# nurturenature/jepsen-tigerbeetle

Measured on AMD Instinct MI355X. Metric: histories/sec, 10k-op/64-proc cas-register histories (time-to-verdict ms in extra), higher is better.
Workload: dtype u64

## Files before the change

### jepsen-tigerbeetle_amd/csrc/batch_create.hip

```cpp
#include "tbc_batch.h"
#include "reach_table.h"

using namespace tbc;

namespace tbc {

uint64_t open_list_entries(const tbc_ops& c, uint64_t op_off, uint64_t n, uint32_t n_events, uint32_t n_slots,
                                  std::vector<uint32_t>& pre, bool branch_lists) {
  const uint64_t worst = std::max<uint64_t>(n, 1) * std::max(1u, n_slots);
  if (n == 0) return 1;
  if ((uint64_t)n_events > 64 * n + 1024) return worst;
  const uint32_t* inv = c.inv_pos + op_off;
  const uint32_t* ret = c.ret_pos + op_off;
  pre.assign((size_t)n_events + 1, 0u);
  for (uint64_t i = 0; i < n; i++) {
    if (ret[i] == TBC_POS_CRASHED) continue;
    if (ret[i] >= n_events || inv[i] > ret[i]) return worst;
    pre[ret[i] + 1] = 1;
  }
  for (uint32_t x = 1; x <= n_events; x++) pre[x] += pre[x - 1];
  uint64_t total = 0;
  const uint8_t* f = c.f + op_off;
  for (uint64_t i = 0; i < n; i++)
    if (ret[i] != TBC_POS_CRASHED && !(branch_lists && f[i] == TBC_F_READ)) total += pre[ret[i]] - pre[inv[i]] + 1;
// ... 354 lines not shown
    }
  }
  if (B->sweep) { tot.bstack_n = 0; tot.btab_n = 0; }
  return TBC_OK;
}

}

void tbc_batch::count_device_bytes() {
  tbc_batch* const B = this;
  const bool beam = B->width > 1;
  B->device_bytes = B->d_f.bytes() + B->d_a.bytes() + B->d_b.bytes() + B->d_proc.bytes() + B->d_inv.bytes() +
                    B->d_ret.bytes() + B->d_hist.bytes() + B->d_rec.bytes() + B->d_seg.bytes() + B->d_ret_slot.bytes() +
                    B->d_ret_op.bytes() + B->d_bitmap.bytes() + B->d_wpre.bytes() + B->d_frames.bytes() +
                    B->d_tab.bytes() + B->d_results.bytes() + B->d_work.bytes() + B->d_witness.bytes();
  if (beam) B->device_bytes += B->d_bh.bytes() + B->d_off.bytes() + B->d_ncr.bytes() + B->d_lst.bytes() +
                               B->d_crashed.bytes() + B->d_slot8.bytes() + B->d_rk8.bytes() + B->d_twn.bytes() + B->d_rdm.bytes() + B->d_look.bytes() + B->d_looktmp.bytes() + B->d_dstack.bytes() + B->d_stack.bytes() + B->d_btab.bytes() + B->d_pool.bytes() + B->d_cmem.bytes();
  if (B->d_stage[0].p) B->device_bytes += B->d_stage[0].bytes();
  if (B->d_stage[1].p) B->device_bytes += B->d_stage[1].bytes();
}

tbc_batch::~tbc_batch() {
  tbc::stream_release(this);
  d_f.release(); d_a.release(); d_b.release(); d_proc.release(); d_inv.release(); d_ret.release();
  d_hist.release(); d_rec.release(); d_seg.release(); d_ret_slot.release(); d_ret_op.release();
  d_bitmap.release(); d_wpre.release(); d_frames.release(); d_witness.release(); d_work.release();
  d_queue.release(); d_tab.release(); d_results.release(); d_table.release(); d_pool_vals.release(); d_cfg.release();
  d_bh.release(); d_off.release(); d_ncr.release(); d_lst.release(); d_crashed.release(); d_stack.release();
  d_zncr.release(); d_reach.release(); d_reach_hdr.release(); d_abort.release(); d_order.release(); d_park.release();
  if (abort_one) (void)hipHostFree(abort_one);
  if (progress) (void)hipHostFree(progress);
  d_progress.release();
  if (!borrowed) { for (auto& e : ev2) if (e) (void)hipEventDestroy(e); if (stream2) (void)hipStreamDestroy(stream2); }
  d_cmem.release(); d_occ.release(); d_btab.release(); d_slot8.release(); d_rk8.release(); d_look.release(); d_looktmp.release(); d_twn.release(); d_rdm.release(); d_cuts.release(); d_seglist.release(); d_sres.release(); d_dstack.release(); d_pool.release(); d_pool_cursor.release();
  if (ev_turn) (void)hipEventDestroy(ev_turn);
  if (!borrowed) {
    for (auto& e : ev) if (e) (void)hipEventDestroy(e);
    if (stream) (void)hipStreamDestroy(stream);
  }
}

namespace tbc {
namespace {

tbc_status alloc_arenas(CreatePlan& P) {
  tbc_batch* B = P.B; const tbc_opts* opts = P.opts; const tbc_model* model = P.model;
  const uint32_t nh = P.nh;
  const bool beam = P.beam, device_sizing = P.device_sizing;
  const LayoutTotals& t = P.tot;
  const uint32_t EW = B->entry_words();
  tbc_status s;
  const uint64_t T = B->total_ops;
  if (!t_ctx) {
    HIP_TRY(hipHostMalloc((void**)&B->progress, 16 * sizeof(uint32_t), hipHostMallocMapped | hipHostMallocCoherent));
    std::memset(B->progress, 0, 16 * sizeof(uint32_t));
    if ((s = B->d_progress.alloc(1))) return s;
  }
  if ((s = B->d_f.alloc(T)) || (s = B->d_a.alloc(T)) || (s = B->d_b.alloc(T)) || (s = B->d_proc.alloc(T)) ||
      (s = B->d_inv.alloc(T)) || (s = B->d_ret.alloc(T)) || (s = B->d_hist.alloc(nh)) || (s = B->d_bh.alloc(beam ? nh : 0)) || (s = B->d_work.alloc(nh)) ||
      (s = B->d_bitmap.alloc(t.bm_n)) || (s = B->d_off.alloc(beam ? t.boff_n : 0)) || (s = B->d_ncr.alloc(beam ? t.boff_n : 0)) || (s = B->d_pool_cursor.alloc(1)) ||
      (s = B->d_rec.alloc(t.rec_n)) ||
      (s = B->d_seg.alloc(t.seg_n)) || (s = B->d_ret_slot.alloc(T)) || (s = B->d_ret_op.alloc(T)) ||
      (s = B->d_wpre.alloc(t.bm_n)) || (s = B->d_frames.alloc(t.frame_n)) ||
      (s = B->d_tab.alloc(t.tab_n)) || (s = B->d_results.alloc(nh)) ||
      (s = B->d_queue.alloc(4)) || (s = B->d_witness.alloc(opts->want_witness ? T : 0)))
    return s;
  if (beam) {
    if ((!device_sizing && (s = B->d_lst.alloc(t.blst_n))) || (s = B->d_crashed.alloc((B->count_form || !B->any_crashed) ? 0 : T)) || (s = B->d_cmem.alloc(B->count_form ? t.bocc_n : 0)) ||
        (s = B->d_slot8.alloc(slot8_bytes(T, nh))) || (s = B->d_stack.alloc(t.bstack_n)) || (s = B->d_btab.alloc(t.btab_n * B->tab_stride())))
      return s;
    if ((B->sweep || B->rsweep) && ((s = B->d_cuts.alloc((uint64_t)nh * B->max_segs)) || (s = B->d_sres.alloc((uint64_t)nh * B->max_segs * kSweepSlices)) || (s = B->d_seglist.alloc((uint64_t)nh * B->max_segs * kSweepSlices * 3)))) return s;
    if (B->sweep || B->rsweep) B->seg_host.resize((size_t)nh * B->max_segs * kSweepSlices);
    if (B->rsweep) {
      std::vector<uint32_t> reach, hdr;
      for (uint32_t h = 0; h < nh; h++) {
        const CountHist& ch = B->count_hist[h];
        hdr.push_back((uint32_t)reach.size());
        hdr.push_back(build_reach_table(ch.words.data(), ch.n_classes, reach));
      }
      if ((s = B->d_zncr.alloc(t.boff_n)) || (s = B->d_reach.alloc(reach.size())) || (s = B->d_reach_hdr.alloc(hdr.size())) || (s = B->d_abort.alloc(nh))) return s;
      HIP_TRY(hipMemset(B->d_zncr.p, 0, B->d_zncr.bytes()));
      HIP_TRY(hipMemcpy(B->d_reach.p, reach.data(), reach.size() * 4, hipMemcpyHostToDevice));
      HIP_TRY(hipMemcpy(B->d_reach_hdr.p, hdr.data(), hdr.size() * 4, hipMemcpyHostToDevice));
      HIP_TRY(hipHostMalloc((void**)&B->abort_one, sizeof(uint32_t), hipHostMallocDefault));
      *B->abort_one = 1u;
    }
    if (B->lanes && (s = B->d_rk8.alloc(slot8_bytes(T, nh)))) return s;
    if (B->reg_rules() && ((!device_sizing && (s = B->d_twn.alloc(t.blst_n * B->mask_words))) || (s = B->d_rdm.alloc(B->lanes ? 1 : T * B->vpad * B->mask_words)))) return s;
    if (B->lanes) { B->d_rdm.release(); if ((s = B->d_rdm.alloc(T * B->front_words()))) return s; }
    const bool by_front = B->mask_words == 1 && B->vpad <= 32;
    if (B->lookahead && ((s = B->d_look.alloc(look_words(T, nh, B->mask_words))) || (s = B->d_looktmp.alloc(by_front ? 0 : T)) ||
                         (s = B->d_dstack.alloc(t.bstack_n)))) return s;
    {
      uint64_t biggest = 0;
      for (uint32_t h = 0; h < nh; h++) biggest = std::max<uint64_t>(biggest, 1ull << B->bh[h].tab_log2);
      uint64_t words = std::max<uint64_t>(t.btab_n * B->tab_stride() * (B->lanes ? 1u : 3u) / 10, biggest * (4 + 16 + 4) * (EW + 1));
      words = std::min<uint64_t>(words, (32ull << 30) / 8);
      if (B->sweep) words = 1;
      if ((s = B->d_pool.alloc(words))) return s;
    }
  }
  if ((s = B->d_cfg.alloc((uint64_t)nh * kCfgCap * (2 + B->mask_words)))) return s;
  if (beam && (s = B->d_park.alloc((uint64_t)nh * kParkWords))) return s;
  B->pool_len = P.desc->cols.pool ? P.desc->cols.pool_len : 0;
  if ((s = B->d_pool_vals.alloc(B->pool_len))) return s;
  if (B->pool_len) HIP_TRY(hipMemcpy(B->d_pool_vals.p, P.desc->cols.pool, (size_t)B->pool_len * 4, hipMemcpyHostToDevice));
  if (model->kind == TBC_MODEL_TABLE) {
    const size_t tn = (size_t)model->n_states * model->n_classes;
    B->table_host.assign(model->table, model->table + tn);
    if ((s = B->d_table.alloc(tn))) return s;
    HIP_TRY(hipMemcpy(B->d_table.p, B->table_host.data(), tn * 2, hipMemcpyHostToDevice));
    B->model.table = nullptr;
  }
  B->count_device_bytes();
  return TBC_OK;
}

tbc_status take_streams(tbc_batch* B) {
  if (t_ctx) {
// ... 236 lines not shown
```

### jepsen-tigerbeetle_amd/csrc/batch_run.hip

```cpp
#include "tbc_batch.h"
#include "witness_expand.h"

using namespace tbc;

namespace tbc {

static SearchArgs make_search_args(tbc_batch* B, uint64_t* tab, uint32_t n_work) {
  SearchArgs a{};
  a.hist = B->d_hist.p; a.rec = B->d_rec.p; a.seg = B->d_seg.p; a.ret_slot = B->d_ret_slot.p;
  a.ret_op = B->d_ret_op.p;
  a.frames = B->d_frames.p; a.tab = tab; a.results = B->d_results.p;
  a.witness = B->opts.want_witness ? B->d_witness.p : nullptr;
  a.work = B->d_work.p; a.queue = B->d_queue.p;
  a.table = B->d_table.p; a.n_work = n_work; a.model_kind = B->model.kind;
  a.init_state = B->model.init;
  a.n_classes = B->model.n_classes; a.n_states = B->model.n_states;
  a.max_steps = B->opts.max_steps;
  a.time_limit_ticks = B->opts.time_limit_ms * 100000ull;
  a.dbg = debug_words();
  a.pool_vals = B->d_pool_vals.p;
  a.cfg = B->d_cfg.p;
  a.progress = B->progress; a.progress_dev = B->d_progress.p;
  return a;
}
// ... 293 lines not shown
    o.algorithm = TBC_ALG_COMPETITION; o.want_witness = 0; o.search_width = 0; o.lanes_per_history = 0; o.round_budget = 0; o.max_steps = 0;
    o.visited_per_op = 0; o.list_order = TBC_ORDER_DEFAULT;
    if (chunk == 1) {
      tbc_ops one = d.cols;
      one.n = (uint32_t)T; one.n_events = nev[0]; one.n_process = npr[0];
      tbc_model m1 = B->model;
      m1.init = aux[0];
      tbc_result r1;
      st = tbc_check(&one, &m1, &o, &r1);
      if (st == TBC_OK) { out[list[lo]] = r1; out[list[lo]].witness = nullptr; tbc_result_free(&r1); }
      continue;
    }
    tbc_batch* I = nullptr;
    st = tbc_batch_create(&d, &B->model, &o, &I);
    if (st == TBC_OK) {
      std::vector<tbc_result> res(k);
      st = tbc_batch_run(I, res.data());
      for (uint32_t i = 0; i < k && st == TBC_OK; i++) { out[list[lo + i]] = res[i]; out[list[lo + i]].witness = nullptr; }
      tbc_batch_destroy(I);
    }
  }
  return st;
}

namespace {

struct RunState {
  tbc_batch* const B;
  tbc_result* const results;
  const int phase;
  const uint64_t t_start;
  const uint32_t nh;
  hipStream_t const s;
  const bool beam;
  const uint32_t KW, EW;
  HostBuf<Hist>& hist_back;
  HostBuf<BeamHist>& bh_back;
  const uint64_t count_budget;
  const uint64_t restart_budget;
  uint64_t first_budget() const { return count_budget ? count_budget : restart_budget; }
  SweepArgs swa{};
  const bool stall_on;
  std::vector<tbc_result> handed;
  std::vector<uint8_t> was_handed;
  std::vector<uint32_t> rs_level;
  std::vector<uint8_t> rs_valid;
  const uint64_t max_bytes;
  std::vector<uint32_t> final_log2;
  std::vector<uint8_t> is_seq;
  std::vector<uint8_t> by_sweep;
  std::vector<uint32_t> width_of;
  std::vector<uint8_t> scratched;
  bool touched_work = false;
  static constexpr uint64_t arena_budget = 32ull << 30;

  RunState(tbc_batch* b, tbc_result* res, int ph)
      : B(b), results(res), phase(ph), t_start(now_ns()), nh(b->n_hist), s(b->stream), beam(b->width > 1), KW(1 + b->mask_words), EW(b->entry_words()),
        hist_back(b->hist_back_m), bh_back(b->bh_back_m),
        count_budget((b->count_form && b->opts.max_steps == 0) ? 32ull * b->max_ops : 0ull),
        restart_budget((ph == 0 && !b->sweep && b->order_restarts_apply()) ? 32ull * b->max_ops : 0ull),
        stall_on(b->lanes != 0 && (b->opts.dominance & TBC_DOM_STALL_HANDOVER) != 0 && !b->count_form && b->mask_words == 1 && !b->opts.want_witness && b->opts.max_steps == 0 && ph == 0 &&
                 (b->model.kind == TBC_MODEL_REGISTER || b->model.kind == TBC_MODEL_CAS_REGISTER) && b->vpad != 0),
        was_handed(b->n_hist, 0), rs_level(b->n_hist, kInf), rs_valid(b->n_hist, 0),
        max_bytes(b->opts.max_visited_bytes ? b->opts.max_visited_bytes : (1ull << 30)) {
    if (B->sweep || B->rsweep) {
      swa.hist = B->d_hist.p; swa.bh = B->d_bh.p; swa.off = B->d_off.p; swa.ncr = B->d_ncr.p; swa.lst = B->d_lst.p;
      swa.crashed = B->d_crashed.p; swa.twn = B->reg_rules() ? B->d_twn.p : nullptr; swa.rdm = B->reg_rules() ? B->d_rdm.p : nullptr;
      swa.slot8 = B->d_slot8.p; swa.cuts = B->d_cuts.p; swa.seg = B->d_sres.p; swa.table = B->d_table.p;
      swa.pool_vals = B->d_pool_vals.p; swa.n_hist = nh; swa.max_segs = B->max_segs; swa.seg_target = B->seg_target;
      swa.cut_open = B->cut_open; swa.n_dom = B->n_dom; swa.vpad = B->vpad ? B->vpad : 1; swa.rules = B->rules;
      swa.model_kind = B->model.kind; swa.init_state = B->model.init;
      swa.n_classes = B->model.n_classes; swa.n_keys = B->model.n_keys;
      swa.shard_rank = 0; swa.shard_world = 1;
    }
  }
};

tbc_status queue_pack(RunState& R) {
  tbc_batch* B = R.B; hipStream_t s = R.s; const uint32_t nh = R.nh; const bool beam = R.beam;
  bool packed = false, counted = false;
  if (nh <= 8) {
    bool fits = true, fits2 = beam;
    for (uint32_t h = 0; h < nh; h++) {
      fits = fits && pack_one_fits(B->model.kind, B->hist[h].n_ops, B->hist[h].n_events, B->hist[h].n_slots);
      fits2 = fits2 && pack_one_counts_fits(B->model.kind, B->hist[h].n_ops, B->hist[h].n_events, B->hist[h].n_slots);
    }
    if (fits2) packed = counted = launch_pack_one_counts(make_pack_args(B), make_pack_open_args(B), s);
    if (!packed && fits) packed = launch_pack_one(make_pack_args(B), s);
  }
  if (!packed && beam) {
    bool fits = true, slots64 = true;
    for (uint32_t h = 0; h < nh && fits; h++) {
      fits = pack_wg_fits(B->model.kind, B->hist[h].n_ops, B->hist[h].n_events, B->hist[h].n_slots);
      slots64 = slots64 && pack_wg64_fits(B->model.kind, B->hist[h].n_ops, B->hist[h].n_events, B->hist[h].n_slots);
    }
    if (fits) packed = counted = launch_pack_wg(make_pack_args(B), make_pack_open_args(B), s, slots64);
  }
  if (!packed) launch_pack(make_pack_args(B), s);
  HIP_TRY(hipGetLastError());
  if (beam) {
    PackOpenArgs po = make_pack_open_args(B);
    if (B->assign_lists) {
      if (!counted) { launch_open_counts(po, s); HIP_TRY(hipGetLastError()); counted = true; }
      tbc_status as = stream_assign_lists(B);
      if (as != TBC_OK) return as;
    }
    launch_pack_open(po, s, counted);
    HIP_TRY(hipGetLastError());
  }
  return TBC_OK;
}

tbc_status first_pass(RunState& R) {
  tbc_batch* B = R.B; hipStream_t s = R.s; const uint32_t nh = R.nh; const bool beam = R.beam; const int phase = R.phase;
  HostBuf<Hist>& hist_back = R.hist_back; HostBuf<BeamHist>& bh_back = R.bh_back;
  TRACE("run: begin");
  HIP_TRY(hipEventRecord(B->ev[0], s));
  if (B->d_progress.p) HIP_TRY(hipMemsetAsync(B->d_progress.p, 0, sizeof(uint32_t), s));
  const bool zero_block = B->borrowed && !guard_on() && !B->d_bitmap.owned && !B->d_off.owned && !B->d_ncr.owned && !B->d_pool_cursor.owned &&
                          (char*)B->d_bitmap.p < (char*)B->d_pool_cursor.p && (size_t)((char*)B->d_pool_cursor.p - (char*)B->d_bitmap.p) < (64u << 20) &&
                          (char*)B->d_off.p > (char*)B->d_bitmap.p && (char*)B->d_off.p < (char*)B->d_pool_cursor.p &&
                          (char*)B->d_ncr.p > (char*)B->d_bitmap.p && (char*)B->d_ncr.p < (char*)B->d_pool_cursor.p;
  const bool fresh = B->inputs_fresh;
  B->inputs_fresh = false;
  if (zero_block) HIP_TRY(hipMemsetAsync(B->d_bitmap.p, 0, (size_t)((char*)B->d_pool_cursor.p - (char*)B->d_bitmap.p) + sizeof(unsigned long long), s));
  else HIP_TRY(hipMemsetAsync(B->d_bitmap.p, 0, B->d_bitmap.bytes(), s));
  const bool use_epoch = beam && B->lanes != 0;
  if (beam) {
    if (use_epoch) B->epoch = B->epoch % 255u + 1u;
    if (!B->sweep && (!use_epoch || B->epoch == 1u)) HIP_TRY(hipMemsetAsync(B->d_btab.p, 0, B->d_btab.bytes(), s));
    if (!B->sweep) HIP_TRY(hipMemsetAsync(B->d_pool.p, 0, B->d_pool.bytes(), s));
    if (!zero_block) {
      HIP_TRY(hipMemsetAsync(B->d_pool_cursor.p, 0, sizeof(unsigned long long), s));
      HIP_TRY(hipMemsetAsync(B->d_off.p, 0, B->d_off.bytes(), s));
      HIP_TRY(hipMemsetAsync(B->d_ncr.p, 0, B->d_ncr.bytes(), s));
    }
    if (!fresh) HIP_TRY(hipMemcpyAsync(B->d_bh.p, B->bh.data(), nh * sizeof(BeamHist), hipMemcpyHostToDevice, s));
  } else {
    HIP_TRY(hipMemsetAsync(B->d_tab.p, 0, B->d_tab.bytes(), s));
  }
  if (!fresh) HIP_TRY(hipMemcpyAsync(B->d_hist.p, B->hist.data(), nh * sizeof(Hist), hipMemcpyHostToDevice, s));
  HIP_TRY(hipEventRecord(B->ev[1], s));
  TRACE("run: memsets queued");
  SYNC_TRACE("memsets");

  if (!B->hist_order.empty()) {
    if (B->d_order.n < nh) { B->d_order.release(); const tbc_status os = B->d_order.alloc(nh); if (os != TBC_OK) return os; }
    HIP_TRY(hipMemcpyAsync(B->d_order.p, B->hist_order.data(), (size_t)nh * 4, hipMemcpyHostToDevice, s));
  }
  tbc_status ps = queue_pack(R);
  if (ps != TBC_OK) return ps;
  TRACE("run: pack launched");
  SYNC_TRACE("pack");
  HIP_TRY(hipEventRecord(B->ev[2], s));

  bool rs_on = B->rsweep && phase == 0 && beam && !B->lanes;
  SweepArgs ra = R.swa;
  if (rs_on) {
    ra.ncr = B->d_zncr.p; ra.crashed = nullptr; ra.reach = B->d_reach.p; ra.reach_hdr = B->d_reach_hdr.p;
    ra.rules = B->rules & (kRuleEager | kRuleTwin);
    HIP_TRY(hipMemsetAsync(B->d_abort.p, 0, B->d_abort.bytes(), s));
    HIP_TRY(hipEventRecord(B->ev2[0], s));
    HIP_TRY(hipStreamWaitEvent(B->stream2, B->ev2[0], 0));
    hist_back.resize(nh);
    if (launch_sweep(ra, B->stream2)) {
      HIP_TRY(hipGetLastError());
      HIP_TRY(hipMemcpyAsync(B->seg_host.data(), B->d_sres.p, B->seg_host.size() * sizeof(SegResult), hipMemcpyDeviceToHost, B->stream2));
      HIP_TRY(hipMemcpyAsync(hist_back.data(), B->d_hist.p, nh * sizeof(Hist), hipMemcpyDeviceToHost, B->stream2));
    } else rs_on = false;
  }

  if (B->sweep) {
    SweepArgs mine = R.swa;
    if (phase == 1 && B->shard_world > 1) {
      mine.shard_rank = B->shard_rank; mine.shard_world = B->shard_world;
      HIP_TRY(hipMemsetAsync(B->d_sres.p, 0, B->d_sres.bytes(), s));
    }
    if (!launch_sweep(mine, s)) { set_error("level sweep launch failed"); return TBC_ERR_HIP; }
  } else if (beam) {
    BeamArgs ba = make_beam_args(B, B->d_btab.p, B->d_stack.p, B->d_dstack.p, nh);
    if (R.first_budget()) ba.max_steps = R.first_budget();
    if (rs_on) ba.abort = B->d_abort.p;
    if (B->lanes) { ba.tab_stride = B->tab_stride(); ba.epoch = use_epoch ? B->epoch : 0u; }
    if (R.stall_on) ba.stall_checks = kStallChecks;
    if (B->lanes) {
      SearchTurn turn(B->device, s);
      if (!B->ev_turn) HIP_TRY(hipEventCreate(&B->ev_turn));
      HIP_TRY(hipEventRecord(B->ev_turn, s));
      if (!launch_narrow(ba, B->mask_words, B->lanes, s, narrow_waves_per_simd())) { set_error("unsupported mask width"); return TBC_ERR_UNSUPPORTED; }
    } else if (!launch_beam(ba, B->mask_words, search_blocks(nh), s)) { set_error("unsupported mask width"); return TBC_ERR_UNSUPPORTED; }
  } else {
    SearchArgs sa = make_search_args(B, B->d_tab.p, nh);
    if (!launch_search(sa, B->mask_words, search_blocks(nh), s)) { set_error("unsupported mask width"); return TBC_ERR_UNSUPPORTED; }
  }
  HIP_TRY(hipGetLastError());
  TRACE("run: search launched");
  SYNC_TRACE("search");
  if (rs_on) {
    HIP_TRY(hipStreamSynchronize(B->stream2));
    const uint32_t SL = kSweepSlices;
    std::vector<uint32_t> again;
    for (uint32_t h = 0; h < nh; h++) if (hist_back[h].status == 0)
      for (uint32_t k = 0; k < B->max_segs; k++) for (uint32_t j = 0; j < SL; j++)
        if (B->seg_host[((size_t)h * B->max_segs + k) * SL + j].status == kSegOverflow) { again.push_back(h); again.push_back(k); again.push_back(j); }
    if (!again.empty()) {
      HIP_TRY(hipMemcpyAsync(B->d_seglist.p, again.data(), again.size() * 4, hipMemcpyHostToDevice, B->stream2));
      SweepArgs r2 = ra;
      r2.seg_list = B->d_seglist.p; r2.n_list = (uint32_t)(again.size() / 3);
      if (launch_sweep(r2, B->stream2)) {
        HIP_TRY(hipGetLastError());
        HIP_TRY(hipMemcpyAsync(B->seg_host.data(), B->d_sres.p, B->seg_host.size() * sizeof(SegResult), hipMemcpyDeviceToHost, B->stream2));
      }
      HIP_TRY(hipStreamSynchronize(B->stream2));
    }
    for (uint32_t h = 0; h < nh; h++) {
      if (hist_back[h].status != 0 || hist_back[h].n_ret == 0) continue;
      tbc_sweep_verdict v{};
      (void)tbc_sweep_compose(&B->seg_host[(size_t)h * B->max_segs * SL], B->max_segs, hist_back[h].n_ret, &v);
      if (v.valid == TBC_INVALID) {
        R.rs_level[h] = v.fail_level;
        HIP_TRY(hipMemcpyAsync(B->d_abort.p + h, B->abort_one, 4, hipMemcpyHostToDevice, B->stream2));
      }
      R.rs_valid[h] = v.valid == TBC_VALID;
    }
    TRACE("run: relaxed sweep composed");
  }
  HIP_TRY(hipEventRecord(B->ev[3], s));
  if (!B->sweep) HIP_TRY(hipMemcpyAsync(B->res_host.data(), B->d_results.p, nh * sizeof(DevResult), hipMemcpyDeviceToHost, s));
  else HIP_TRY(hipMemcpyAsync(B->seg_host.data(), B->d_sres.p, B->seg_host.size() * sizeof(SegResult), hipMemcpyDeviceToHost, s));
  hist_back.resize(nh);
  bh_back.resize(beam ? nh : 0);
  HIP_TRY(hipMemcpyAsync(hist_back.data(), B->d_hist.p, nh * sizeof(Hist), hipMemcpyDeviceToHost, s));
  if (beam) HIP_TRY(hipMemcpyAsync(bh_back.data(), B->d_bh.p, nh * sizeof(BeamHist), hipMemcpyDeviceToHost, s));
  if (B->borrowed && B->sweep) {
    const uint64_t t_spin = now_ns();
    hipError_t q;
    while ((q = hipStreamQuery(s)) == hipErrorNotReady && now_ns() - t_spin < 3000000ull) {}
    if (q != hipSuccess && q != hipErrorNotReady) HIP_TRY(q);
  }
  HIP_TRY(hipStreamSynchronize(s));
  if (rs_on) HIP_TRY(hipStreamSynchronize(B->stream2));
  TRACE("run: first pass synced");
  for (uint32_t h = 0; h < nh; h++) if (R.rs_level[h] != kInf) {
    DevResult& d = B->res_host[h];
    std::memset(&d, 0, sizeof d);
    d.valid = TBC_UNKNOWN; d.cause = TBC_CAUSE_STEP_LIMIT; d.fail_op = TBC_NO_OP; d.prev_ok_op = TBC_NO_OP; d.final_state = B->model.init;
    d.tab_log2 = B->bh[h].tab_log2;
  }
  return TBC_OK;
}

tbc_status sweep_verdicts(RunState& R) {
  tbc_batch* B = R.B; hipStream_t s = R.s; const uint32_t nh = R.nh;
  HostBuf<Hist>& hist_back = R.hist_back; HostBuf<BeamHist>& bh_back = R.bh_back;
  const SweepArgs& swa = R.swa;
  const uint32_t SL = kSweepSlices;
  {
    std::vector<uint32_t> again;
    for (uint32_t h = 0; h < nh; h++) if (hist_back[h].status == 0 && bh_back[h].status == 0)
      for (uint32_t k = 0; k < B->max_segs; k++) for (uint32_t j = 0; j < SL; j++)
        if (B->seg_host[((size_t)h * B->max_segs + k) * SL + j].status == kSegOverflow) { again.push_back(h); again.push_back(k); again.push_back(j); }
    if (!again.empty()) {
      HIP_TRY(hipMemcpyAsync(B->d_seglist.p, again.data(), again.size() * 4, hipMemcpyHostToDevice, s));
      SweepArgs sa2 = swa;
      sa2.seg_list = B->d_seglist.p; sa2.n_list = (uint32_t)(again.size() / 3);
      if (launch_sweep(sa2, s)) {
        HIP_TRY(hipGetLastError());
        HIP_TRY(hipMemcpyAsync(B->seg_host.data(), B->d_sres.p, B->seg_host.size() * sizeof(SegResult), hipMemcpyDeviceToHost, s));
      }
      HIP_TRY(hipStreamSynchronize(s));
    }
  }
  std::vector<uint32_t> fb, lg;
  for (uint32_t h = 0; h < nh; h++) {
    DevResult& d = B->res_host[h];
    std::memset(&d, 0, sizeof d);
    d.fail_op = TBC_NO_OP; d.prev_ok_op = TBC_NO_OP; d.final_state = B->model.init;
    if (hist_back[h].status != 0) { d.valid = TBC_UNKNOWN; continue; }
    if (hist_back[h].n_ret == 0) { d.valid = TBC_VALID; R.by_sweep[h] = 1; continue; }
    const SegResult* sg = &B->seg_host[(size_t)h * B->max_segs * SL];
    tbc_sweep_verdict v{};
    (void)tbc_sweep_compose(sg, B->max_segs, hist_back[h].n_ret, &v);
    const bool give_up = bh_back[h].status != 0 || v.valid == TBC_UNKNOWN;
    const uint32_t fail_seg = v.valid == TBC_INVALID ? v.fail_seg : kInf, fail_level = v.fail_level;
    const bool ended = v.valid == TBC_VALID;
    const uint32_t* live_in = v.live_in;
    d.steps = v.probes; d.probes = v.probes; d.visited = v.configs_total; d.backtracks = v.subrounds; d.max_depth = v.max_level;
    if (std::getenv("TBC_DEBUG")) {
      uint32_t longest = 0; uint64_t maxp = 0;
      for (uint32_t q = 0; q < B->max_segs * SL; q++) if (sg[q].status == kSegOk) { longest = std::max(longest, sg[q].F1 - sg[q].F0); maxp = std::max<uint64_t>(maxp, sg[q].probes); }
      std::fprintf(stderr, "[tbc sweep] history %u: %u wavefronts, longest segment %u levels, most probes in one %llu, largest level %llu, verdict %d\n",
                   h, v.n_wavefronts, longest, (unsigned long long)maxp, (unsigned long long)v.max_level, v.valid);
    }
    if (give_up || (fail_seg == kInf && !ended)) { fb.push_back(h); lg.push_back(B->bh[h].tab_log2); continue; }
    R.by_sweep[h] = 1;
// ... 146 lines not shown
  }
  return TBC_OK;
}

static const uint32_t kRestartOrders[] = {16u + 48u, 2u, 1u, 16u + 8u, 0u};

static const uint32_t kRaceOrders[] = {16u + 48u, 2u, 1u, 16u + 8u, 0u};
tbc_status race_orders(RunState& R, const std::vector<uint32_t>& pend_all) {
  tbc_batch* B = R.B; const uint32_t nh = R.nh; hipStream_t s = R.s;
  constexpr uint32_t K = sizeof(kRaceOrders) / sizeof(kRaceOrders[0]);
  const uint32_t default_order = B->list_order();
  R.handed.resize(nh);
  B->last_raced = (uint32_t)pend_all.size();
  CtxSuspend own_arenas;
  size_t mem_free = 0, mem_total = 0;
  if (hipMemGetInfo(&mem_free, &mem_total) != hipSuccess) mem_free = 32ull << 30;
  const uint64_t mem_cap = std::max<uint64_t>(8ull << 30, (uint64_t)mem_free / 4 * 3);
  std::vector<DevResult> outer_res(nh);
  size_t lo = 0;
  while (lo < pend_all.size()) {
    uint64_t ops = 0;
    size_t hi = lo;
    while (hi < pend_all.size() && (hi == lo || (ops + B->hist[pend_all[hi]].n_ops) * 4000ull * (K + 1) <= mem_cap)) { ops += B->hist[pend_all[hi]].n_ops; hi++; }
    const uint32_t k = (uint32_t)(hi - lo);
    std::vector<uint32_t> res_list, outer_map(nh, 0u);
    for (uint32_t i = 0; i < k; i++) {
      const uint32_t h = pend_all[lo + i];
      outer_map[h] = i;
      if (!R.scratched[h] && B->d_park.p) res_list.push_back(h);
    }
    DevBuf<uint32_t> decided, d_outer_map, d_inner_map;
    tbc_status st;
    if ((st = decided.alloc(k)) || (st = d_outer_map.alloc(nh))) return st;
    HIP_TRY(hipMemsetAsync(decided.p, 0, (size_t)k * 4, s));
    HIP_TRY(hipMemcpyAsync(d_outer_map.p, outer_map.data(), (size_t)nh * 4, hipMemcpyHostToDevice, s));
    std::vector<uint32_t> rep_hist, rep_order;
    for (uint32_t i = 0; i < k; i++) {
      for (uint32_t o : kRaceOrders) if (o != default_order) { rep_hist.push_back(i); rep_order.push_back(o); }
      if (R.scratched[pend_all[lo + i]] || !B->d_park.p) { rep_hist.push_back(i); rep_order.push_back(default_order); }
    }
    const uint32_t nr = (uint32_t)rep_hist.size();
    FetchedColumns fc;
    if ((st = fetch_columns(B, pend_all.data() + lo, k, fc)) != TBC_OK) return st;
    const std::vector<uint64_t>& goff = fc.off;
    const uint8_t* const gf = fc.f; const int32_t* const ga = fc.a; const int32_t* const gb = fc.b; const int32_t* const gp = fc.proc;
    const uint32_t* const gi = fc.inv; const uint32_t* const gr = fc.ret;
    const uint32_t n_res = (uint32_t)res_list.size();
    if (n_res) {
      HIP_TRY(hipMemcpyAsync(B->d_work.p, res_list.data(), (size_t)n_res * 4, hipMemcpyHostToDevice, s));
      BeamArgs ba = make_beam_args(B, B->d_btab.p, B->d_stack.p, B->d_dstack.p, n_res);
      ba.resume = 1; ba.max_steps = 0; ba.abort = decided.p; ba.abort_set = decided.p; ba.abort_map = d_outer_map.p;
      if (!launch_beam(ba, B->mask_words, search_blocks(n_res), s)) { set_error("unsupported mask width"); return TBC_ERR_UNSUPPORTED; }
      HIP_TRY(hipGetLastError());
      R.touched_work = true;
    }
    std::vector<uint64_t> off(nr + 1, 0);
    std::vector<uint32_t> nev(nr), npr(nr), imap(nr);
    for (uint32_t r = 0; r < nr; r++) {
      const Hist& H = B->hist[pend_all[lo + rep_hist[r]]];
      off[r + 1] = off[r] + H.n_ops; nev[r] = H.n_events; npr[r] = H.n_slots; imap[r] = rep_hist[r];
    }
    const uint64_t T = off[nr];
    if (T > 0xFFFFFFFFull) { set_error("the race's replicas exceed 2^32 ops"); return TBC_ERR_OOM; }
    std::vector<uint8_t> f(T + 1);
    std::vector<int32_t> a(T + 1), b(T + 1), pr(T + 1);
    std::vector<uint32_t> inv(T + 1), ret(T + 1);
    for (uint32_t r = 0; r < nr; r++) {
      const uint64_t n = off[r + 1] - off[r], o = off[r], g0 = goff[rep_hist[r]];
      std::memcpy(f.data() + o, gf + g0, n);
      std::memcpy(a.data() + o, ga + g0, n * 4); std::memcpy(b.data() + o, gb + g0, n * 4); std::memcpy(pr.data() + o, gp + g0, n * 4);
      std::memcpy(inv.data() + o, gi + g0, n * 4); std::memcpy(ret.data() + o, gr + g0, n * 4);
    }
    tbc_batch_desc d{};
    d.n_hist = nr; d.op_off = off.data(); d.n_events = nev.data(); d.n_process = npr.data();
    d.cols.n = (uint32_t)T; d.cols.f = f.data(); d.cols.a = a.data(); d.cols.b = b.data(); d.cols.process = pr.data();
    d.cols.inv_pos = inv.data(); d.cols.ret_pos = ret.data();
    tbc_opts o = B->opts;
    o.algorithm = TBC_ALG_COMPETITION; o.want_witness = 0; o.search_width = B->width; o.lanes_per_history = 64; o.round_budget = 0; o.max_steps = 0;
    o.visited_per_op = 64; o.list_order = TBC_ORDER_SLOT; o.dominance = (B->opts.dominance | TBC_DOM_NO_ORDER_RESTARTS) & ~TBC_DOM_STALL_HANDOVER;
    std::vector<tbc_result> res(nr);
    tbc_batch* inner = nullptr;
    TRACE("race: the replicas' batch is being made");
    st = nr ? tbc_batch_create(&d, &B->model, &o, &inner) : TBC_OK;
    if (st == TBC_OK && nr) {
      st = d_inner_map.alloc(nr);
      if (st == TBC_OK && hipMemcpy(d_inner_map.p, imap.data(), (size_t)nr * 4, hipMemcpyHostToDevice) != hipSuccess) st = TBC_ERR_HIP;
      if (st == TBC_OK) {
        inner->ext_abort = decided.p; inner->ext_abort_set = decided.p; inner->ext_abort_map = d_inner_map.p;
        inner->hist_order = rep_order;
        TRACE("race: the replicas run");
        st = tbc_batch_run(inner, res.data());
        TRACE("race: the replicas are done");
      }
    }
    if (inner) tbc_batch_destroy(inner);
    HIP_TRY(hipSetDevice(B->device));
    const bool inner_ok = nr != 0 && (st == TBC_OK || st == TBC_ERR_BAD_HISTORY || st == TBC_ERR_MODEL);
    if (!inner_ok && n_res == 0) { decided.release(); d_outer_map.release(); d_inner_map.release(); return st == TBC_OK ? TBC_ERR_HIP : st; }
    if (n_res) HIP_TRY(hipMemcpyAsync(outer_res.data(), B->d_results.p, (size_t)nh * sizeof(DevResult), hipMemcpyDeviceToHost, s));
    HIP_TRY(hipStreamSynchronize(s));
    TRACE("race: the resumed default order is done");
    decided.release(); d_outer_map.release(); d_inner_map.release();
    std::vector<uint32_t> first_rep(k, 0xFFFFFFFFu);
    for (uint32_t r = nr; r-- > 0;) first_rep[rep_hist[r]] = r;
    for (uint32_t i = 0; i < k; i++) {
      const uint32_t h = pend_all[lo + i];
// ... 325 lines not shown
```

### jepsen-tigerbeetle_amd/csrc/tbc_batch.h

```cpp
#pragma once
#include <hip/hip_runtime.h>
#include <algorithm>
#include <atomic>
#include <chrono>
#include <cstdio>
#include <cstdlib>
#include <cstring>
#include <deque>
#include <mutex>
#include <new>
#include <thread>
#include <vector>
#include "tbc_internal.h"

namespace tbc {

#define HIP_TRY(expr)                                                             \
  do {                                                                            \
    hipError_t e_ = (expr);                                                       \
    if (e_ != hipSuccess) {                                                       \
      ::tbc::set_error("%s failed: %s (%s:%d)", #expr, hipGetErrorString(e_), __FILE__, __LINE__); \
      return e_ == hipErrorOutOfMemory ? TBC_ERR_OOM : TBC_ERR_HIP;               \
    }                                                                             \
  } while (0)

inline uint32_t ceil_log2(uint64_t x) {
  uint32_t l = 0;
  while ((1ull << l) < x) l++;
  return l;
}

uint64_t now_ns();
bool device_is_gfx950(int dev);
uint32_t* debug_words();
#define SYNC_TRACE(msg) do { if (std::getenv("TBC_SYNC_EACH")) { hipError_t e__ = hipStreamSynchronize(s); std::fprintf(stderr, "[tbc sync] %s -> %s\n", msg, hipGetErrorString(e__)); std::fflush(stderr); } } while (0)
#define TRACE(msg) do { if (std::getenv("TBC_DEBUG")) { std::fprintf(stderr, "[tbc %9.3f ms] %s\n", (double)(::tbc::now_ns() % 100000000000ull) / 1e6, msg); std::fflush(stderr); } } while (0)

struct Ctx {
  int device = 0;
  char* slab = nullptr;
  size_t cap = 0, used = 0, wanted = 0;
  char* pin = nullptr;
  size_t pin_cap = 0, pin_used = 0, pin_wanted = 0;
  hipStream_t stream = nullptr;
  hipEvent_t ev[6] = {};
  hipStream_t stream2 = nullptr;
  hipEvent_t ev2[2] = {};
};
extern thread_local Ctx* t_ctx;
Ctx* ctx_acquire(int device);
void ctx_release(Ctx* c);
struct CtxSuspend {
  Ctx* const saved;
  CtxSuspend() : saved(t_ctx) { t_ctx = nullptr; }
  ~CtxSuspend() { t_ctx = saved; }
};

bool guard_on();
constexpr size_t kGuardBytes = 256;
extern thread_local const void* t_guard_owner;
extern thread_local size_t t_guard_nth;
void guard_add(const void* arena_end);
void guard_remove(const void* arena_end);
size_t guard_check(const char* when, const void* owner);

template <typename T>
// ... 130 lines not shown
  std::vector<uint32_t> hist_order;
  tbc::DevBuf<uint32_t> d_order;
  tbc::DevBuf<uint32_t> d_park;
  uint32_t last_raced = 0;
  uint32_t* progress = nullptr;
  tbc::DevBuf<uint32_t> d_progress;
  mutable std::atomic<uint32_t> progress_seen{0};
  std::atomic<uint64_t> run_t0{0};
  std::atomic<uint32_t> running{0};
  bool order_restarts_apply() const {
    return width > 1 && !lanes && !count_form && list_order_applies() && opts.list_order == TBC_ORDER_DEFAULT && opts.max_steps == 0 &&
           !(opts.dominance & TBC_DOM_NO_ORDER_RESTARTS);
  }
  std::vector<tbc::BeamHist> bh;
  tbc::DevBuf<tbc::BeamHist> d_bh;
  tbc::DevBuf<uint32_t> d_off, d_ncr, d_stack;
  tbc::DevBuf<tbc::OpRec> d_lst, d_crashed;
  tbc::DevBuf<uint8_t> d_slot8;
  tbc::DevBuf<uint8_t> d_rk8;
  bool lookahead = false;
  tbc::DevBuf<uint64_t> d_look;
  tbc::DevBuf<uint32_t> d_dstack;
  tbc::DevBuf<uint32_t> d_looktmp;
  bool sweep = false;
  uint32_t max_segs = 1, seg_target = 0, cut_open = 0, n_dom = 1;
  tbc::DevBuf<uint32_t> d_cuts, d_seglist;
  tbc::DevBuf<tbc::SegResult> d_sres;
  tbc::HostBuf<tbc::SegResult> seg_host;
  bool rsweep = false;
  tbc::DevBuf<uint32_t> d_zncr, d_reach, d_reach_hdr, d_abort;
  hipStream_t stream2 = nullptr;
  hipEvent_t ev2[2] = {};
  uint32_t* abort_one = nullptr;
  uint32_t last_segments = 0, last_fallback = 0;
  uint32_t shard_rank = 0, shard_world = 1;
  bool partial_done = false;
  tbc::HostBuf<tbc::Hist> hist_back_m;
  tbc::HostBuf<tbc::BeamHist> bh_back_m;
  tbc::HostBuf<char> upload_stage;
  bool inputs_fresh = false;
  uint32_t rules = 0;
  uint32_t vpad = 0;
  tbc::DevBuf<uint64_t> d_twn, d_rdm;
  tbc::DevBuf<uint64_t> d_occ, d_btab, d_pool;
  bool count_form = false;
  tbc::DevBuf<uint64_t> d_cmem;
  std::vector<tbc::CountHist> count_hist;
  uint32_t reg_rules() const { return rules & (tbc::kRuleEager | tbc::kRuleTwin); }
  uint32_t epoch = 0;
  bool any_crashed = true;
  uint32_t tab_stride() const { return entry_words() - ((lanes && !opts.want_witness) ? 1u : 0u); }
  uint32_t entry_words() const { return mask_words + 2u + (count_form ? tbc::kCountWords : 0u); }
  tbc::DevBuf<unsigned long long> d_pool_cursor;
  std::vector<tbc::DevResult> res_host;
  std::vector<uint32_t> witness_host;
  uint64_t timing_ns[4] = {0, 0, 0, 0};
  hipEvent_t ev_turn = nullptr;
  uint64_t turn_wait_ns = 0;
  tbc_counters sum{};
  uint64_t device_bytes = 0;
  void count_device_bytes();

  struct InputSlot { char* mem = nullptr; size_t bytes = 0; hipEvent_t copied = nullptr; bool busy = false; uint32_t* planned = nullptr; };
  std::vector<InputSlot> in_slots;
  uint32_t in_hist_cap = 0;
  uint64_t in_ops_cap = 0;
  tbc::DevBuf<uint32_t> d_stage[2];
  hipStream_t stream_copy = nullptr;
  hipEvent_t ev_stage[2] = {};
  hipEvent_t ev_unpacked[2] = {};
  bool stage_used[2] = {false, false};
  uint64_t in_seq = 0;
  std::deque<tbc_pending_input> pending;
  tbc::DevBuf<uint32_t> d_in_flags;
  uint32_t* in_flags_host = nullptr;
  bool assign_lists = false;
  tbc::DevBuf<uint32_t> d_list_over;
  uint64_t in_bytes_copied = 0, in_copy_ns = 0;
  hipEvent_t ev_copy[2][2] = {};
  tbc::LayoutTotals cap;
  bool lists_headroom = false;
  bool inputs_stale = false;
  uint64_t inputs_consumed = 0;
  uint32_t lists_regrown = 0, reload_slot = 0;

  bool borrowed = false;
  ~tbc_batch();
};

namespace tbc {

struct ColumnScan { bool nonneg = true, any_crashed = false, any_crashed_effect = false; int32_t vmax = -1; };
ColumnScan scan_columns(const tbc_ops& c, uint64_t T);
tbc_status layout_histories(tbc_batch* B, uint32_t nh, const uint64_t* op_off, const uint32_t* n_events, const uint32_t* n_slots, const int32_t* aux,
                            const uint32_t* list_caps, bool lists_on_device, std::vector<Hist>& hist, std::vector<BeamHist>& bh, LayoutTotals& tot,
                            const std::vector<CountHist>* count_hist = nullptr);
bool build_count_form(const tbc_ops& c, uint64_t o0, uint64_t n, uint32_t n_process, bool cas_model, int32_t* slot_col, CountHist& out,
                      std::vector<uint32_t>& rets, std::vector<int32_t>& slot_of, std::vector<uint8_t>& used);
uint64_t open_list_entries(const tbc_ops& c, uint64_t op_off, uint64_t n, uint32_t n_events, uint32_t n_slots, std::vector<uint32_t>& pre, bool branch_lists);
tbc_status batch_create_impl(const tbc_batch_desc* desc, const tbc_model* model, const tbc_opts* opts, tbc_batch* B);

PackArgs make_pack_args(tbc_batch* B);
PackOpenArgs make_pack_open_args(tbc_batch* B);
tbc_status batch_run_impl(tbc_batch* B, tbc_result* results, int phase = 0);

tbc_status stream_consume(tbc_batch* B, bool* consumed);
// ... 6 lines not shown
```

Baseline: 380,400.

## Trim per-pass device memsets using memoized pool usage and dirty tracking

Replaces the unconditional per-run memsets of the bitmap, offsets, ncr and visited pool with a planner. The bitmap and offsets are cleared only when the pack kernel does not already overwrite them. ncr is cleared only when the previous pass may have dirtied it. The pool is cleared only up to the cursor value read back from the previous pass. The progress word now lives next to the pool cursor, so a single memset resets both. This cuts redundant device fill bandwidth and launch count, at the cost of extra host-side state that must be kept correct across timeouts, races and arena changes.

```diff
diff --git a/jepsen-tigerbeetle_amd/csrc/batch_create.hip b/jepsen-tigerbeetle_amd/csrc/batch_create.hip
--- a/jepsen-tigerbeetle_amd/csrc/batch_create.hip
+++ b/jepsen-tigerbeetle_amd/csrc/batch_create.hip
@@ -430,19 +430,20 @@
   tbc_status s;
   const uint64_t T = B->total_ops;
   if (!t_ctx) {
-    HIP_TRY(hipHostMalloc((void**)&B->progress, 16 * sizeof(uint32_t), hipHostMallocMapped | hipHostMallocCoherent));
-    std::memset(B->progress, 0, 16 * sizeof(uint32_t));
-    if ((s = B->d_progress.alloc(1))) return s;
+    HIP_TRY(hipHostMalloc((void**)&B->progress, 18 * sizeof(uint32_t), hipHostMallocMapped | hipHostMallocCoherent));
+    std::memset(B->progress, 0, 18 * sizeof(uint32_t));
+    B->pool_used_host = reinterpret_cast<unsigned long long*>(B->progress + 16);
   }
   if ((s = B->d_f.alloc(T)) || (s = B->d_a.alloc(T)) || (s = B->d_b.alloc(T)) || (s = B->d_proc.alloc(T)) ||
       (s = B->d_inv.alloc(T)) || (s = B->d_ret.alloc(T)) || (s = B->d_hist.alloc(nh)) || (s = B->d_bh.alloc(beam ? nh : 0)) || (s = B->d_work.alloc(nh)) ||
-      (s = B->d_bitmap.alloc(t.bm_n)) || (s = B->d_off.alloc(beam ? t.boff_n : 0)) || (s = B->d_ncr.alloc(beam ? t.boff_n : 0)) || (s = B->d_pool_cursor.alloc(1)) ||
+      (s = B->d_bitmap.alloc(t.bm_n)) || (s = B->d_off.alloc(beam ? t.boff_n : 0)) || (s = B->d_ncr.alloc(beam ? t.boff_n : 0)) || (s = B->d_pool_cursor.alloc(t_ctx ? 1 : 2)) ||
       (s = B->d_rec.alloc(t.rec_n)) ||
       (s = B->d_seg.alloc(t.seg_n)) || (s = B->d_ret_slot.alloc(T)) || (s = B->d_ret_op.alloc(T)) ||
       (s = B->d_wpre.alloc(t.bm_n)) || (s = B->d_frames.alloc(t.frame_n)) ||
       (s = B->d_tab.alloc(t.tab_n)) || (s = B->d_results.alloc(nh)) ||
       (s = B->d_queue.alloc(4)) || (s = B->d_witness.alloc(opts->want_witness ? T : 0)))
     return s;
+  if (!t_ctx) { B->d_progress.p = reinterpret_cast<uint32_t*>(B->d_pool_cursor.p + 1); B->d_progress.n = 1; B->d_progress.owned = false; B->d_progress.guarded = false; }
   if (beam) {
     if ((!device_sizing && (s = B->d_lst.alloc(t.blst_n))) || (s = B->d_crashed.alloc((B->count_form || !B->any_crashed) ? 0 : T)) || (s = B->d_cmem.alloc(B->count_form ? t.bocc_n : 0)) ||
         (s = B->d_slot8.alloc(slot8_bytes(T, nh))) || (s = B->d_stack.alloc(t.bstack_n)) || (s = B->d_btab.alloc(t.btab_n * B->tab_stride())))
diff --git a/jepsen-tigerbeetle_amd/csrc/batch_run.hip b/jepsen-tigerbeetle_amd/csrc/batch_run.hip
--- a/jepsen-tigerbeetle_amd/csrc/batch_run.hip
+++ b/jepsen-tigerbeetle_amd/csrc/batch_run.hip
@@ -369,6 +369,7 @@
   std::vector<uint32_t> width_of;
   std::vector<uint8_t> scratched;
   bool touched_work = false;
+  bool block_zeroed = false;
   static constexpr uint64_t arena_budget = 32ull << 30;
 
   RunState(tbc_batch* b, tbc_result* res, int ph)
@@ -413,8 +414,11 @@
     }
     if (fits) packed = counted = launch_pack_wg(make_pack_args(B), make_pack_open_args(B), s, slots64);
   }
+  const PackFills pf = plan_pack_fills(R.block_zeroed, beam, packed, counted);
+  if (pf.bitmap) HIP_TRY(hipMemsetAsync(B->d_bitmap.p, 0, B->d_bitmap.bytes(), s));
   if (!packed) launch_pack(make_pack_args(B), s);
   HIP_TRY(hipGetLastError());
+  if (pf.off) HIP_TRY(hipMemsetAsync(B->d_off.p, 0, B->d_off.bytes(), s));
   if (beam) {
     PackOpenArgs po = make_pack_open_args(B);
     if (B->assign_lists) {
@@ -433,7 +437,6 @@
   HostBuf<Hist>& hist_back = R.hist_back; HostBuf<BeamHist>& bh_back = R.bh_back;
   TRACE("run: begin");
   HIP_TRY(hipEventRecord(B->ev[0], s));
-  if (B->d_progress.p) HIP_TRY(hipMemsetAsync(B->d_progress.p, 0, sizeof(uint32_t), s));
   const bool zero_block = B->borrowed && !guard_on() && !B->d_bitmap.owned && !B->d_off.owned && !B->d_ncr.owned && !B->d_pool_cursor.owned &&
                           (char*)B->d_bitmap.p < (char*)B->d_pool_cursor.p && (size_t)((char*)B->d_pool_cursor.p - (char*)B->d_bitmap.p) < (64u << 20) &&
                           (char*)B->d_off.p > (char*)B->d_bitmap.p && (char*)B->d_off.p < (char*)B->d_pool_cursor.p &&
@@ -441,17 +444,19 @@
   const bool fresh = B->inputs_fresh;
   B->inputs_fresh = false;
   if (zero_block) HIP_TRY(hipMemsetAsync(B->d_bitmap.p, 0, (size_t)((char*)B->d_pool_cursor.p - (char*)B->d_bitmap.p) + sizeof(unsigned long long), s));
-  else HIP_TRY(hipMemsetAsync(B->d_bitmap.p, 0, B->d_bitmap.bytes(), s));
+  R.block_zeroed = zero_block;
+  if (!zero_block) HIP_TRY(hipMemsetAsync(B->d_pool_cursor.p, 0, B->d_pool_cursor.bytes(), s));
   const bool use_epoch = beam && B->lanes != 0;
   if (beam) {
     if (use_epoch) B->epoch = B->epoch % 255u + 1u;
     if (!B->sweep && (!use_epoch || B->epoch == 1u)) HIP_TRY(hipMemsetAsync(B->d_btab.p, 0, B->d_btab.bytes(), s));
-    if (!B->sweep) HIP_TRY(hipMemsetAsync(B->d_pool.p, 0, B->d_pool.bytes(), s));
-    if (!zero_block) {
-      HIP_TRY(hipMemsetAsync(B->d_pool_cursor.p, 0, sizeof(unsigned long long), s));
-      HIP_TRY(hipMemsetAsync(B->d_off.p, 0, B->d_off.bytes(), s));
-      HIP_TRY(hipMemsetAsync(B->d_ncr.p, 0, B->d_ncr.bytes(), s));
-    }
+    FillFacts ff;
+    ff.one_memset = zero_block; ff.lists = true; ff.has_pool = !B->sweep; ff.writes_ncr = B->any_crashed;
+    ff.epoch_wrapped = use_epoch && B->epoch == 1u;
+    ff.ncr_arena = B->d_ncr.p; ff.ncr_words = B->d_ncr.n; ff.pool_arena = B->d_pool.p; ff.pool_words = B->d_pool.n;
+    const FillPlan fp = plan_pass_fills(ff, B->fill_memo);
+    if (fp.pool_words) HIP_TRY(hipMemsetAsync(B->d_pool.p, 0, (size_t)fp.pool_words * sizeof(uint64_t), s));
+    if (fp.ncr) HIP_TRY(hipMemsetAsync(B->d_ncr.p, 0, B->d_ncr.bytes(), s));
     if (!fresh) HIP_TRY(hipMemcpyAsync(B->d_bh.p, B->bh.data(), nh * sizeof(BeamHist), hipMemcpyHostToDevice, s));
   } else {
     HIP_TRY(hipMemsetAsync(B->d_tab.p, 0, B->d_tab.bytes(), s));
@@ -549,6 +554,8 @@
   bh_back.resize(beam ? nh : 0);
   HIP_TRY(hipMemcpyAsync(hist_back.data(), B->d_hist.p, nh * sizeof(Hist), hipMemcpyDeviceToHost, s));
   if (beam) HIP_TRY(hipMemcpyAsync(bh_back.data(), B->d_bh.p, nh * sizeof(BeamHist), hipMemcpyDeviceToHost, s));
+  const bool cursor_back = beam && !B->sweep && B->pool_used_host != nullptr;
+  if (cursor_back) HIP_TRY(hipMemcpyAsync(B->pool_used_host, B->d_pool_cursor.p, sizeof(unsigned long long), hipMemcpyDeviceToHost, s));
   if (B->borrowed && B->sweep) {
     const uint64_t t_spin = now_ns();
     hipError_t q;
@@ -558,6 +565,12 @@
   HIP_TRY(hipStreamSynchronize(s));
   if (rs_on) HIP_TRY(hipStreamSynchronize(B->stream2));
   TRACE("run: first pass synced");
+  if (cursor_back) {
+    bool timed_out = false;
+    for (uint32_t h = 0; h < nh && !timed_out; h++) timed_out = B->res_host[h].valid == TBC_UNKNOWN && B->res_host[h].cause == TBC_CAUSE_TIME_LIMIT;
+    B->fill_memo.pool_known = !timed_out;
+    B->fill_memo.pool_used = *B->pool_used_host;
+  }
   for (uint32_t h = 0; h < nh; h++) if (R.rs_level[h] != kInf) {
     DevResult& d = B->res_host[h];
     std::memset(&d, 0, sizeof d);
@@ -810,6 +823,7 @@
       ba.resume = 1; ba.max_steps = 0; ba.abort = decided.p; ba.abort_set = decided.p; ba.abort_map = d_outer_map.p;
       if (!launch_beam(ba, B->mask_words, search_blocks(n_res), s)) { set_error("unsupported mask width"); return TBC_ERR_UNSUPPORTED; }
       HIP_TRY(hipGetLastError());
+      B->fill_memo.pool_known = false;
       R.touched_work = true;
     }
     std::vector<uint64_t> off(nr + 1, 0);
diff --git a/jepsen-tigerbeetle_amd/csrc/pass_fills.h b/jepsen-tigerbeetle_amd/csrc/pass_fills.h
--- /dev/null
+++ b/jepsen-tigerbeetle_amd/csrc/pass_fills.h
@@ -0,0 +1,66 @@
+#pragma once
+#include <cstdint>
+
+namespace tbc {
+
+struct FillMemo {
+  bool ncr_dirty = true;
+  bool pool_known = false;
+  uint64_t pool_used = 0;
+  const void* ncr_arena = nullptr;
+  uint64_t ncr_words = 0;
+  const void* pool_arena = nullptr;
+  uint64_t pool_words = 0;
+};
+
+struct FillFacts {
+  bool one_memset = false;
+  bool lists = false;
+  bool has_pool = false;
+  bool writes_ncr = false;
+  bool epoch_wrapped = false;
+  const void* ncr_arena = nullptr;
+  uint64_t ncr_words = 0;
+  const void* pool_arena = nullptr;
+  uint64_t pool_words = 0;
+};
+
+struct FillPlan {
+  bool ncr = false;
+  uint64_t pool_words = 0;
+};
+
+struct PackFills {
+  bool bitmap = false, off = false;
+};
+inline PackFills plan_pack_fills(bool one_memset, bool lists, bool lds_pack, bool counts_pack) {
+  PackFills p;
+  p.bitmap = !one_memset && !lds_pack;
+  p.off = !one_memset && lists && !counts_pack;
+  return p;
+}
+
+inline FillPlan plan_pass_fills(const FillFacts& f, FillMemo& m) {
+  FillPlan p;
+  if (f.one_memset) {
+    p.pool_words = f.has_pool ? f.pool_words : 0;
+    m = FillMemo{};
+    return p;
+  }
+  if (f.lists) {
+    const bool ncr_new = m.ncr_arena != f.ncr_arena || m.ncr_words != f.ncr_words;
+    p.ncr = m.ncr_dirty || ncr_new;
+    m.ncr_arena = f.ncr_arena; m.ncr_words = f.ncr_words;
+    m.ncr_dirty = f.writes_ncr;
+  }
+  if (f.has_pool) {
+    const bool pool_new = m.pool_arena != f.pool_arena || m.pool_words != f.pool_words;
+    const bool whole = pool_new || f.epoch_wrapped || !m.pool_known;
+    p.pool_words = whole ? f.pool_words : (m.pool_used < f.pool_words ? m.pool_used : f.pool_words);
+    m.pool_arena = f.pool_arena; m.pool_words = f.pool_words;
+  }
+  m.pool_known = false; m.pool_used = 0;
+  return p;
+}
+
+}
diff --git a/jepsen-tigerbeetle_amd/csrc/tbc_batch.h b/jepsen-tigerbeetle_amd/csrc/tbc_batch.h
--- a/jepsen-tigerbeetle_amd/csrc/tbc_batch.h
+++ b/jepsen-tigerbeetle_amd/csrc/tbc_batch.h
@@ -12,6 +12,7 @@
 #include <thread>
 #include <vector>
 #include "tbc_internal.h"
+#include "pass_fills.h"
 
 namespace tbc {
 
@@ -248,6 +249,8 @@
   uint32_t tab_stride() const { return entry_words() - ((lanes && !opts.want_witness) ? 1u : 0u); }
   uint32_t entry_words() const { return mask_words + 2u + (count_form ? tbc::kCountWords : 0u); }
   tbc::DevBuf<unsigned long long> d_pool_cursor;
+  tbc::FillMemo fill_memo;
+  unsigned long long* pool_used_host = nullptr;
   std::vector<tbc::DevResult> res_host;
   std::vector<uint32_t> witness_host;
   uint64_t timing_ns[4] = {0, 0, 0, 0};
```

After: 383,200 (median of 6 runs). Within noise of the previous version (+0.7%).
